# thomasahle/tinyknn

Measured on AMD Instinct MI355X. Metric: queries/sec at Recall10@10 on GloVe-100 angular (synthetic stand-in), IVF+4-bit PQ, build_probes=1, higher is better.
Workload: dtype int8 (saturating PQ sums) + f32 (tables, rescoring)

## Files before the change

include/tinyknn_hip.h:

```cpp
#ifndef TINYKNN_HIP_H
#define TINYKNN_HIP_H

#include <stdint.h>

#ifdef __cplusplus
extern "C" {
#endif

#define TK_ORDER_SSE 0
#define TK_ORDER_AVX 1

#define TK_OK 0
#define TK_ERR_ARG (-1)
#define TK_ERR_HIP (-2)
#define TK_ERR_STATE (-3)

const char *tk_last_error(void);
int tk_version(void);
int tk_device_count(void);
int tk_set_device(int device);


int tk_estimate_pq(const uint64_t *data, int64_t chunks, int M, const uint64_t *tables,
                   uint64_t *out, int signd, int order);
// ... 58 lines not shown
                             int q_pq_is_f64, int64_t nq, int k, int n_probes, int pass_1,
                             int64_t *out_ids_dev, void *stream);

int tk_index_set_pipeline(tk_index *ix, int depth);
int tk_index_join(tk_index *ix, void *stream);
int tk_index_set_coalesce(tk_index *ix, int n);
int tk_index_quiesce(tk_index *ix);

int tk_index_set_heap_mode(tk_index *ix, int mode);

int tk_index_set_scan_mode(tk_index *ix, int mode);

int tk_index_set_plain_scan(tk_index *ix, int mode);
int tk_index_plain_stats(tk_index *ix, int64_t *out8);
#define TK_OPT_SCAN_FORM 1
#define TK_OPT_RESCORE_FORM 2
#define TK_OPT_PLAIN_LIMIT 3
#define TK_OPT_REPLAY_LAZY 4
#define TK_OPT_REPLAY_COUNT 5
#define TK_OPT_REPLAY_TWIN 6
#define TK_OPT_TWIN_VOUCH 7
#define TK_OPT_PAIR_NQ 8
#define TK_OPT_LABELS24 9
int tk_index_set_option(tk_index *ix, int option, int value);
int tk_index_twin_table(tk_index *ix, int64_t *rows, int *w, int32_t *list_out, int32_t *off_out);

int tk_index_set_profiling(tk_index *ix, int on);
int tk_index_last_profile(tk_index *ix, float *ms8, double *scan_bytes, int *batches);

int tk_index_replay_stats(tk_index *ix, int64_t *out4);
int tk_measure_read_bandwidth(int64_t bytes, int reps, double *gbps);
int tk_measure_gather_bandwidth(int64_t table_bytes, int row_bytes, int64_t n_gather, int reps, double *gbps);
int tk_scan_exclusive_host(const void *in_host, void *out_host, int64_t n, int is64);

float *tk_index_alloc_data(tk_index *ix, int64_t N, int d);
int tk_index_synth_data(tk_index *ix, int64_t row0, int64_t n, uint64_t seed, const float *centres,
                        int n_centres, float sigma);
int tk_synth_rows(float *out, int64_t row0, int64_t n, int d, uint64_t seed, const float *centres,
                  int n_centres, float sigma);
int tk_index_build_dev(tk_index *ix, int normalise, const float *all_centers,
                       const float *search_centers, const float *ynorm2, int64_t C, int n_probes,
                       const double *R, int d_pad, int64_t *n_active_out);
int tk_index_export_lists(tk_index *ix, int64_t *list_sizes, uint64_t *codes, int64_t *ids);
int tk_index_export_centers(tk_index *ix, float *active_centers, uint64_t *center_codes);
int tk_index_read_rows(tk_index *ix, const int64_t *rows, int64_t n, float *out);

// ... 89 lines not shown
```

tinyknn_amd/_lib.py:

```python
import ctypes as C
import os

_HERE = os.path.dirname(os.path.abspath(__file__))

ORDER_SSE, ORDER_AVX = 0, 1


class TinyKnnHipError(RuntimeError):
    pass


def lib_path():
    return os.environ.get("TINYKNN_HIP_LIB", os.path.join(_HERE, "libtinyknn_hip.so"))


_lib = None
_lib_pid = None

_i64p = C.POINTER(C.c_int64)
_i32p = C.POINTER(C.c_int32)
_u64p = C.POINTER(C.c_uint64)
_u8p = C.POINTER(C.c_uint8)
_f32p = C.POINTER(C.c_float)
_f64p = C.POINTER(C.c_double)

OPT_SCAN_FORM, OPT_RESCORE_FORM, OPT_PLAIN_LIMIT, OPT_REPLAY_LAZY, OPT_REPLAY_COUNT, OPT_REPLAY_TWIN, OPT_TWIN_VOUCH = 1, 2, 3, 4, 5, 6, 7
OPT_PAIR_NQ, OPT_LABELS24 = 8, 9

SIGNATURES = {
    "tk_last_error": (C.c_char_p, []),
    "tk_version": (C.c_int, []),
    "tk_device_count": (C.c_int, []),
    "tk_set_device": (C.c_int, [C.c_int]),
    "tk_estimate_pq": (C.c_int, [_u64p, C.c_int64, C.c_int, _u64p, _u64p, C.c_int, C.c_int]),
    "tk_estimate_pq_batch": (C.c_int, [_u64p, C.c_int64, C.c_int, _u64p, C.c_int64, _u64p,
                                       C.c_int, C.c_int]),
    "tk_query_pq": (C.c_int, [_u64p, C.c_int64, C.c_int, C.c_int64, _u64p, _i64p, _i32p, C.c_int,
                              C.c_int, _i64p, C.c_int]),
    "tk_init_heap": (C.c_int, [_i64p, _i32p, C.c_int, C.c_int]),
    "tk_heap_insert": (C.c_int, [_i64p, _i32p, C.c_int, C.c_int64, C.c_int32]),
    "tk_heap_insert_is": (C.c_int, [_i64p, _i32p, C.c_int, C.c_int64, C.c_int32]),
    "tk_build_tables": (C.c_int, [_f32p, C.c_int, C.c_int, C.c_int, C.c_void_p, C.c_int, C.c_int64,
                                  C.c_double, C.c_double, C.c_int, _u8p, C.c_void_p, _f64p]),
    "tk_knn_brute1": (C.c_int64, [C.c_void_p, C.c_int, C.c_void_p, C.c_int, C.c_int64, C.c_int,
                                  C.c_int64, _i64p]),
    "tk_encode_pq": (C.c_int, [_f32p, C.c_int, C.c_int, C.c_void_p, C.c_int, C.c_int64, _u8p]),
    "tk_assign_lists": (C.c_int, [_f32p, C.c_int64, C.c_int, C.c_int, C.c_void_p, C.c_int,
                                  C.c_void_p, C.c_int64, C.c_int, _i64p]),
    "tk_codes_upload": (C.c_void_p, [_u64p, C.c_int64, C.c_int]),
    "tk_codes_free": (None, [C.c_void_p]),
# ... 151 lines not shown
```

tinyknn_amd/csrc/api_build.hip:

```cpp
#include "api_internal.h"

static int upload_rotation(tk_index *ix, const double *R, int d_pad)
{
    std::vector<double> rt((size_t)d_pad * ix->dq);
    for (int j = 0; j < ix->dq; j++)
        for (int t = 0; t < d_pad; t++) rt[(size_t)t * ix->dq + j] = R[(size_t)j * d_pad + t];
    TRY(ix->rot_t.ensure(rt.size() * 8));
    HIPCHECK(hipMemcpy(ix->rot_t.p, rt.data(), rt.size() * 8, hipMemcpyHostToDevice));
    ix->rot_d_pad = d_pad;
    return TK_OK;
}

extern "C" float *tk_index_alloc_data(tk_index *ix, int64_t N, int d)
{
    IXLOCK(ix);
    if (!ix || !ix->have_pq || N < 1 || d < 1) {
        fail(TK_ERR_ARG, "bad argument: tk_index_alloc_data (set_pq first, N >= 1, d >= 1)");
        return nullptr;
    }
    if (ix->data.ensure((size_t)N * d * 4) != TK_OK) return nullptr;
    ix->N = N;
    ix->d = d;
    ix->data_is_f64 = 0;
    ix->have_data = ix->have_centers = ix->have_lists = false;
    return ix->data.as<float>();
}

static int synth_centres(DevBuf &buf, const float *centres, int n_centres, int d, const float **dev)
{
    *dev = nullptr;
    if (!centres || n_centres <= 0) return TK_OK;
    TRY(buf.ensure((size_t)n_centres * d * 4));
    HIPCHECK(hipMemcpy(buf.p, centres, (size_t)n_centres * d * 4, hipMemcpyHostToDevice));
    *dev = buf.as<float>();
    return TK_OK;
}

extern "C" int tk_index_synth_data(tk_index *ix, int64_t row0, int64_t n, uint64_t seed,
                                   const float *centres, int n_centres, float sigma)
{
    IXLOCK(ix);
    ARGCHECK(ix && ix->data.p && ix->N > 0, "tk_index_alloc_data first");
    ARGCHECK(row0 >= 0 && n >= 0 && row0 + n <= ix->N, "row range");
    const float *cd = nullptr;
    TRY(synth_centres(ix->stage, centres, n_centres, ix->d, &cd));
    tk_launch_synth_rows(ix->data.as<float>() + row0 * ix->d, row0, n, ix->d, seed, cd, n_centres, sigma, 0);
    HIPCHECK(hipGetLastError());
// ... 170 lines not shown
    HIPCHECK(hipMemcpy(ix->ids_off.p, ioff.data(), (size_t)(L + 1) * 8, hipMemcpyHostToDevice));
    HIPCHECK(hipMemcpy(ix->list_n.p, sizes.data(), (size_t)L * 8, hipMemcpyHostToDevice));
    const size_t tiled_bytes = (size_t)tk_tiled_uint4s(coff[(size_t)L], P) * 16;
    TRY(ix->codes.ensure(tiled_bytes));
    HIPCHECK(hipMemset(ix->codes.p, 0, tiled_bytes));
    tk_launch_pack_lists(labels.as<uint8_t>(), M, rows2.as<int>(), ix->ids_off.as<int64_t>(),
                         ix->list_chunk_off.as<int64_t>(), ix->list_n.as<int64_t>(), (int)L, zero_code,
                         ix->codes.as<uint4>(), coff[(size_t)L], 0);
    tk_launch_widen_ids(rows2.as<int>(), T, ix->ids.as<int64_t>(), 0);
    HIPCHECK(hipGetLastError());
    ix->ids_unique = kp == 1;
    ix->labels24 = ix->N < 0x00ffffff;
    ix->have_ids32 = false;
    if (kp > 1) {
        TRY(ix->ids32.ensure((size_t)T * 4));
        HIPCHECK(hipMemcpyAsync(ix->ids32.p, rows2.p, (size_t)T * 4, hipMemcpyDeviceToDevice, 0));
        ix->have_ids32 = true;
    }
    HIPCHECK(hipDeviceSynchronize());
    ix->sharded = false; ix->rank = 0; ix->world = 1;
    ix->total_chunks = coff[(size_t)L];
    ix->total_ids = T;
    ix->max_list_chunks = (int)maxc;
    ix->have_centers = ix->have_lists = ix->have_data = true;
    TRY(build_twins(ix, N));
    if (n_active_out) *n_active_out = L;
    return TK_OK;
}

extern "C" int tk_index_shard_resident(tk_index *ix, const int32_t *owner, int rank, int world)
{
    IXLOCK(ix);
    ARGCHECK(ix && ix->have_lists && !ix->sharded, "a complete unsharded index");
    ARGCHECK(owner && world >= 1 && rank >= 0 && rank < world, "owner / rank / world");
    TRY(flush_pending(ix));
    HIPCHECK(hipDeviceSynchronize());
    const int64_t L = ix->n_lists;
    std::vector<int64_t> sizes((size_t)L), coff((size_t)L + 1, 0), loff((size_t)L + 1, 0);
    HIPCHECK(hipMemcpy(sizes.data(), ix->list_n.p, (size_t)L * 8, hipMemcpyDeviceToHost));
    for (int64_t i = 0; i < L; i++) {
        ARGCHECK(owner[i] >= 0 && owner[i] < world, "owner out of range");
        const int64_t c = (sizes[(size_t)i] + 15) / 16;
        coff[(size_t)i + 1] = coff[(size_t)i] + c;
        loff[(size_t)i + 1] = loff[(size_t)i] + (owner[i] == rank ? c : 0);
    }
    const int P = ix->M / 2;
// ... 36 lines not shown
    ix->n_lists = src->n_lists; ix->center_chunks = src->center_chunks; ix->d = src->d;
    ix->list_chunk_off.borrow(src->list_chunk_off);
    ix->list_n.borrow(src->list_n);
    ix->ids_off.borrow(src->ids_off);
    ix->ids.borrow(src->ids);
    ix->ids32.borrow(src->ids32);
    ix->have_ids32 = src->have_ids32;
    ix->labels24 = src->labels24;
    ix->twin_list.borrow(src->twin_list);
    ix->twin_off.borrow(src->twin_off);
    ix->twin_w = src->twin_w;
    ix->twin_unverified = src->twin_unverified;
    ix->twin_vouched = src->twin_vouched;
    ix->opt_replay_twin = src->opt_replay_twin;
    ix->total_chunks = src->total_chunks; ix->total_ids = src->total_ids;
    ix->max_list_chunks = src->max_list_chunks;
    ix->ids_unique = src->ids_unique;
    ix->cslots_i.borrow(src->cslots_i);
    ix->cslots_l.borrow(src->cslots_l);
    ix->c_chunk_off.borrow(src->c_chunk_off);
    ix->rot_t.borrow(src->rot_t);
    ix->rot_d_pad = src->rot_d_pad;
    ix->data.borrow(src->data);
    ix->N = src->N; ix->data_is_f64 = src->data_is_f64;
    ix->have_pq = ix->have_centers = ix->have_lists = ix->have_data = true;
    ix->plain_mode = src->plain_mode;
    const int64_t L = ix->n_lists;
    std::vector<int64_t> sizes((size_t)L), loff((size_t)L + 1, 0);
    bool ok = hipMemcpy(sizes.data(), src->list_n.p, (size_t)L * 8, hipMemcpyDeviceToHost) == hipSuccess;
    for (int64_t i = 0; ok && i < L; i++) {
        ok = owner[i] >= 0 && owner[i] < world;
        loff[(size_t)i + 1] = loff[(size_t)i] + (owner[i] == rank ? (sizes[(size_t)i] + 15) / 16 : 0);
    }
    const int P = ix->M / 2;
    const size_t bytes = (size_t)tk_tiled_uint4s(loff[(size_t)L], P) * 16;
    ok = ok && ix->owner.ensure((size_t)L * 4) == TK_OK && ix->local_chunk_off.ensure((size_t)(L + 1) * 8) == TK_OK &&
         ix->codes.ensure(bytes > 0 ? bytes : 16) == TK_OK;
    ok = ok && hipMemcpy(ix->owner.p, owner, (size_t)L * 4, hipMemcpyHostToDevice) == hipSuccess &&
         hipMemcpy(ix->local_chunk_off.p, loff.data(), (size_t)(L + 1) * 8, hipMemcpyHostToDevice) == hipSuccess &&
         hipMemset(ix->codes.p, 0, bytes > 0 ? bytes : 16) == hipSuccess;
    if (ok) {
        tk_launch_compact_tiled(src->codes.as<uint4>(), ix->codes.as<uint4>(), P, ix->list_chunk_off.as<int64_t>(),
                                ix->local_chunk_off.as<int64_t>(), (int)L, loff[(size_t)L], 0);
        ok = hipGetLastError() == hipSuccess && hipDeviceSynchronize() == hipSuccess;
    }
    if (!ok) {
// ... 305 lines not shown
```

tinyknn_amd/csrc/api_index.hip:

```cpp
#include "api_internal.h"


struct Pending;
static int batch_epilogue(const struct Pending &b, hipStream_t st);


extern "C" tk_index *tk_index_create(void)
{
    if (require_gpu() != TK_OK) return nullptr;
    tk_index *ix = new tk_index();
    ix->works.resize(1);
    const char *e = getenv("TINYKNN_PLAIN_SCAN");
    if (e && e[0] == '2') ix->plain_mode = 2;
    e = getenv("TINYKNN_PAIR_NQ");
    if (e && e[0] >= '0' && e[0] <= '9') ix->opt_pair_nq = atoi(e);
    return ix;
}

extern "C" void tk_index_destroy(tk_index *ix)
{
    if (!ix) return;
    (void)flush_pending(ix);
    (void)hipDeviceSynchronize();
    DevBuf *bufs[] = {&ix->pq_centers, &ix->active_centers, &ix->center_codes, &ix->list_chunk_off,
                      &ix->list_n, &ix->ids_off, &ix->ids, &ix->codes, &ix->ids32, &ix->data, &ix->cslots_i,
                      &ix->cslots_l, &ix->c_chunk_off, &ix->q, &ix->qpq, &ix->stage, &ix->owner,
                      &ix->local_chunk_off, &ix->rot_t, &ix->br_ynorm, &ix->br_vals, &ix->br_tau,
                      &ix->br_cand, &ix->br_count, &ix->br_out, &ix->br_q, &ix->br_sample, &ix->replay_counters,
                      &ix->twin_list, &ix->twin_off};
    for (DevBuf *b : bufs) b->release();
    for (Work &w : ix->works) w.release();
    if (ix->ev_in) (void)hipEventDestroy(ix->ev_in);
    for (auto &e : ix->evs) (void)hipEventDestroy(e);
    delete ix;
}

extern "C" int tk_index_set_pq(tk_index *ix, const float *centers, int dq, int dpb, int f_order,
                               double sqrt_n_blocks, int order)
{
    IXLOCK(ix);
    ARGCHECK(ix, "null index");
    ARGCHECK(dpb >= 1 && dpb <= 32 && dq % dpb == 0, "dq/dpb");
    ARGCHECK((dq / dpb) % 2 == 0, "number of blocks must be even");
    ARGCHECK(dq / dpb <= 512, "at most 512 blocks");
    ARGCHECK(order == TK_ORDER_SSE || order == TK_ORDER_AVX, "order");
    TRY(ix->pq_centers.ensure((size_t)16 * dq * 4));
    HIPCHECK(hipMemcpy(ix->pq_centers.p, centers, (size_t)16 * dq * 4, hipMemcpyHostToDevice));
    ix->dq = dq; ix->dpb = dpb; ix->M = dq / dpb; ix->f_order = f_order;
    ix->sqrt_nb = sqrt_n_blocks; ix->order = order;
    ix->have_pq = true;
    return TK_OK;
}
// ... 62 lines not shown
    TRY(t.where.ensure((size_t)label_bound * b * 4));
    TRY(ix->twin_list.ensure((size_t)T * w * 4));
    TRY(ix->twin_off.ensure((size_t)T * w * 4));
    HIPCHECK(hipMemsetAsync(t.cnt.p, 0, (size_t)label_bound * 4, 0));
    tk_launch_twin_fill(ix->ids32.as<int32_t>(), T, t.cnt.as<int>(), t.where.as<int>(), b,
                        ix->ids_off.as<int64_t>(), (int)ix->n_lists, ix->twin_list.as<int32_t>(),
                        ix->twin_off.as<int32_t>(), 0);
    HIPCHECK(hipGetLastError());
    HIPCHECK(hipDeviceSynchronize());
    if (!ix->sharded) {
        HIPCHECK(hipMemsetAsync(t.cnt.p, 0, 4, 0));
        tk_launch_twin_verify(ix->codes.as<uint4>(), ix->M / 2, ix->list_chunk_off.as<int64_t>(),
                              ix->ids_off.as<int64_t>(), (int)ix->n_lists, ix->twin_list.as<int32_t>(),
                              ix->twin_off.as<int32_t>(), w, T, t.cnt.as<int>(), 0);
        int bad = 0;
        HIPCHECK(hipMemcpy(&bad, t.cnt.p, 4, hipMemcpyDeviceToHost));
        if (bad) return TK_OK;
    }
    ix->twin_w = w;
    ix->twin_unverified = ix->sharded;
    return TK_OK;
}

int build_twins(tk_index *ix, int64_t label_bound)
{
    ix->twin_w = 0;
    ix->twin_unverified = false;
    ix->twin_list.release();
    ix->twin_off.release();
    const int64_t T = ix->total_ids;
    if (!ix->have_ids32 || ix->ids_unique || T <= 0 || T >= (1ll << 31) || label_bound <= 0 ||
        label_bound > 8 * T + 1024 || ix->n_lists >= (1ll << 31))
        return TK_OK;
    TwinScratch t;
    const int rc = build_twins_try(ix, label_bound, t);
    if (rc != TK_OK || ix->twin_w == 0) {
        ix->twin_w = 0;
        ix->twin_unverified = false;
        ix->twin_list.release();
        ix->twin_off.release();
    }
    if (rc != TK_OK) (void)hipGetLastError();
    return TK_OK;
}

extern "C" int tk_index_twin_table(tk_index *ix, int64_t *rows, int *w, int32_t *list_out, int32_t *off_out)
// ... 105 lines not shown

extern "C" int tk_index_set_lists_shard(tk_index *ix, const int64_t *list_sizes,
                                        const int32_t *owner, int rank, int world,
                                        const uint64_t *codes_owned, const int64_t *ids)
{
    IXLOCK(ix);
    ARGCHECK(owner, "owner");
    ARGCHECK(world >= 1 && rank >= 0 && rank < world, "rank/world");
    return set_lists_impl(ix, list_sizes, codes_owned, ids, owner, rank, world);
}

extern "C" int tk_index_set_data(tk_index *ix, const void *data, int data_is_f64, int64_t N,
                                 int d)
{
    IXLOCK(ix);
    ARGCHECK(ix && ix->have_centers, "set_centers first");
    ARGCHECK(d == ix->d, "data dimension differs from the centres'");
    ARGCHECK(N >= 1, "N");
    const size_t esz = data_is_f64 ? 8 : 4;
    TRY(ix->data.ensure((size_t)N * d * esz));
    HIPCHECK(hipMemcpy(ix->data.p, data, (size_t)N * d * esz, hipMemcpyHostToDevice));
    ix->N = N;
    ix->data_is_f64 = data_is_f64;
    ix->have_data = true;
    return TK_OK;
}


int make_plan(const tk_index *ix, int k, int n_probes, int pass_1, Plan &p)
{
    ARGCHECK(ix && ix->have_pq && ix->have_centers && ix->have_lists && ix->have_data,
             "index not fully populated (pq, centers, lists, data)");
    ARGCHECK(k >= 1 && n_probes >= 1, "k and n_probes must be >= 1");
    int64_t kc = n_probes < ix->n_lists ? n_probes : ix->n_lists;
    int64_t rescore = 2 * kc + 10 < ix->n_lists ? 2 * kc + 10 : ix->n_lists;
    int64_t R = pass_1 > 0 ? pass_1 : (int64_t)(n_probes + 1) * k + 1;
    ARGCHECK(R * 12 + 16 <= 64 * 1024 && rescore * 12 + 16 <= 64 * 1024,
             "heap larger than 64 KiB of LDS (pass_1 <= 5460)");
    ARGCHECK(R * (ix->data_is_f64 ? 16 : 12) + (int64_t)ix->d * (ix->data_is_f64 ? 8 : 4) + 16 <= 64 * 1024,
             "rescoring tile larger than 64 KiB of LDS");
    p.kc = (int)kc; p.rescore = (int)rescore; p.R = (int)R; p.S = (int)kc;
    p.cap = (int64_t)kc * ix->max_list_chunks;
    if (p.cap < 1) p.cap = 1;
    ARGCHECK(p.cap < (1ll << 31), "probed chunk range overflows int32");
    p.cap_min = (p.cap + 15) / 16 * 16;
    p.ccap_min = (ix->center_chunks + 15) / 16 * 16;
// ... 619 lines not shown
                                        slot_loff, p.S, ix->ids.as<int64_t>(),
                                        w.heap_idx.as<int64_t>(), w.heap_val.as<int32_t>(), p.R, 1,
                                        0, plain ? repeat_flag : nullptr, w.mins.as<uint8_t>(), p.cap_min,
                                        ix->ids32.as<int32_t>(), st, slot_exact, qlim))
            return fail(TK_ERR_HIP, "hipFuncSetAttribute(LDS size) failed");
        if (plain) {
            rescan_flagged(ix, w, q0, nq, p, st);
            tk_launch_heap_replay_packed(w.dist.as<uint4>(), p.cap, nq, slot_prefix, slot_n, slot_loff,
                                         p.S, ix->ids.as<int64_t>(), w.heap_idx.as<int64_t>(),
                                         w.heap_val.as<int32_t>(), p.R, 1, 0, repeat_flag, 1, 1, st);
        }
    } else if (packed_ok) {
        tk_launch_heap_replay_packed(w.dist.as<uint4>(), p.cap, nq, slot_prefix, slot_n, slot_loff,
                                     p.S, ix->ids.as<int64_t>(), w.heap_idx.as<int64_t>(),
                                     w.heap_val.as<int32_t>(), p.R, 1, 0, nullptr, 0, 1, st);
    } else {
        tk_launch_heap_fill(w.heap_idx.as<int64_t>(), w.heap_val.as<int32_t>(), nq * p.R, 127, st);
        tk_launch_heap_replay(w.dist.as<uint4>(), p.cap, nq, slot_prefix, slot_n, slot_loff, p.S,
                              ix->ids.as<int64_t>(), w.heap_idx.as<int64_t>(),
                              w.heap_val.as<int32_t>(), p.R, 1, 0, nullptr, st);
    }
    TRY(pf.mark(st));
    tk_launch_rescore(q_dev, 0, ix->d, ix->data.p, ix->data_is_f64, ix->N, w.heap_idx.as<int64_t>(), p.R, nq, k, 1,
                      out_dev, nullptr, st, ix->opt_rescore_form, q2, out2);
    TRY(pf.mark(st));
    return TK_OK;
}

struct Pending {
    Work *w;
    const float *q_dev;
    int64_t nq;
    int k;
    Plan p;
    int64_t *out_dev;
    bool units;
    bool plain;
    bool coarse_launched;
    int64_t *host_out;
    bool host_out_kernel;
    hipEvent_t user_ev;
    Prof pf;
    hipStream_t st, sf, sl;
    struct Sub {
        int64_t *out_dev;
        int64_t nq;
        int64_t *host_out;
// ... 574 lines not shown
{
    IXLOCK(ix);
    ARGCHECK(ix, "null index");
    ARGCHECK(mode >= 0 && mode <= 3, "mode");
    TRY(flush_pending(ix));
    ix->heap_mode = mode;
    return TK_OK;
}

extern "C" int tk_index_set_option(tk_index *ix, int option, int value)
{
    IXLOCK(ix);
    ARGCHECK(ix, "null index");
    TRY(flush_pending(ix));
    switch (option) {
    case TK_OPT_SCAN_FORM:
        ARGCHECK(value >= 0 && value <= 2, "TK_OPT_SCAN_FORM: 0, 1 or 2");
        ix->opt_scan_form = value;
        return TK_OK;
    case TK_OPT_RESCORE_FORM:
        ARGCHECK(value >= 0 && value <= 2, "TK_OPT_RESCORE_FORM: 0, 1 or 2");
        ix->opt_rescore_form = value;
        return TK_OK;
    case TK_OPT_PLAIN_LIMIT:
        ix->opt_plain_limit = value;
        return TK_OK;
    case TK_OPT_PAIR_NQ:
        ARGCHECK(value >= 0, "TK_OPT_PAIR_NQ: >= 0");
        ix->opt_pair_nq = value;
        return TK_OK;
    case TK_OPT_LABELS24:
        ix->opt_labels24 = value != 0;
        return TK_OK;
    case TK_OPT_REPLAY_COUNT:
        ix->opt_replay_count = value != 0;
        if (value) {
            TRY(ix->replay_counters.ensure(64));
            HIPCHECK(hipMemset(ix->replay_counters.p, 0, 64));
        }
        return TK_OK;
    case TK_OPT_REPLAY_LAZY:
        ARGCHECK(value >= -1 && value <= 1, "TK_OPT_REPLAY_LAZY: -1, 0 or 1");
        ix->opt_replay_lazy = value;
        return TK_OK;
    case TK_OPT_REPLAY_TWIN:
        ARGCHECK(value == 0 || value == 1, "TK_OPT_REPLAY_TWIN: 0 or 1");
// ... 137 lines not shown
```

tinyknn_amd/csrc/api_internal.h:

```cpp
#pragma once
#include <algorithm>
#include <cmath>
#include <mutex>
#include <stdlib.h>
#include <string.h>
#include <stdio.h>
#include <string>
#include <vector>

#include "../../include/tinyknn_hip.h"
#include "kernels.h"

int tk_fail(int code, const std::string &msg);
static inline int fail(int code, const std::string &msg) { return tk_fail(code, msg); }

#define HIPCHECK(x)                                                                          \
    do {                                                                                     \
        hipError_t e_ = (x);                                                                 \
        if (e_ != hipSuccess) {                                                              \
            char b_[512];                                                                    \
            snprintf(b_, sizeof b_, "%s failed: %s (%s:%d)", #x, hipGetErrorString(e_),      \
                     __FILE__, __LINE__);                                                    \
            return fail(TK_ERR_HIP, b_);                                                     \
        }                                                                                    \
// ... 131 lines not shown
    DevBuf list_chunk_off, list_n, ids_off, ids, codes, ids32;
    bool have_ids32 = false;
    bool labels24 = false;
    int opt_labels24 = 1;
    DevBuf twin_list, twin_off;
    int twin_w = 0;
    bool twin_unverified = false, twin_vouched = false;
    int opt_replay_twin = 1;
    int64_t total_chunks = 0, total_ids = 0;
    int max_list_chunks = 0;
    bool ids_unique = false;
    int heap_mode = 0;
    int opt_pair_nq = 8192;
    bool have_pq = false, have_centers = false, have_lists = false, have_data = false;
    DevBuf owner, local_chunk_off;
    DevBuf rot_t;
    DevBuf br_ynorm, br_vals, br_tau, br_cand, br_count, br_out, br_q, br_sample;
    int rot_d_pad = 0;
    int rank = 0, world = 1;
    bool sharded = false;
    DevBuf data;
    int64_t N = 0;
    int data_is_f64 = 0;
    DevBuf cslots_i, cslots_l, c_chunk_off, q, qpq, stage;
    int scan_mode = 0;
    int opt_scan_form = 0;
    int opt_rescore_form = 2;
    int opt_plain_limit = 0x7fffffff;
    DevBuf replay_counters;
    bool opt_replay_count = false;
    int opt_replay_lazy = -1;
    bool flat_plain_ok = true;
    int plain_state = 0;
    int plain_skip = 0;
    int plain_backoff = 256;
    int plain_wait = 0;
    bool capturing = false;
    int plain_mode = 0;
    bool host_out_kernel = false;
    std::vector<Work> works;
    int depth = 1;
    uint64_t calls = 0;
    std::vector<hipStream_t> lat_streams;
    hipEvent_t ev_in = nullptr;
    std::vector<struct Pending *> pending;
    uint64_t ev_seq = 0;
// ... 32 lines not shown
    size_t base = 0;
    int evi = 0;
    int set = -1;
    bool plain_marked = false;
    int mark(hipStream_t st)
    {
        if (evs) HIPCHECK(hipEventRecord((*evs)[base + (size_t)evi++], st));
        return TK_OK;
    }
    int mark_plain(int which, hipStream_t st)
    {
        if (evs) {
            HIPCHECK(hipEventRecord((*evs)[base + 8 + (size_t)which], st));
            plain_marked = true;
        }
        return TK_OK;
    }
};

inline const uint4 *tables_of(const Work &w) { return w.tables.as<uint4>(); }

int flush_pending(tk_index *ix);
int build_twins(tk_index *ix, int64_t label_bound);
bool twin_replay(const tk_index *ix, const struct Plan &p);
int make_plan(const tk_index *ix, int k, int n_probes, int pass_1, Plan &p);
bool plain_env_on();
int plain_k(const tk_index *ix, int64_t nq, const Plan &p);
size_t plain_desc_bytes(const tk_index *ix, int64_t nq, const Plan &p);
double workspace_bytes();
bool coarse_units(const tk_index *ix, int64_t nq);
int stage_tables(tk_index *ix, Work &w, const void *qpq_dev, int qpq_f64, int64_t nq, hipStream_t st, Prof &pf,
                 bool plain = false, TkSecond qpq2 = TkSecond(), int64_t row0 = 0);
TkScanJob coarse_job(const tk_index *ix, const Work &w, const Plan &p);
int plain_blocks();
int shard_plain_blocks();
void launch_coarse_scan(tk_index *ix, Work &w, int64_t nq, const Plan &p, hipStream_t st,
                        const uint4 *tables = nullptr);
int coarse_replay_probes(tk_index *ix, Work &w, const float *q_dev, int64_t nq, const Plan &p,
                         int64_t *probes_out, hipStream_t st, Prof &pf, TkSecond q2 = TkSecond(),
                         const TkSlotsOut *slots = nullptr, int *slots_written = nullptr);
void coarse_slots(tk_index *ix, Work &w, const int64_t *probes, int64_t nq, const Plan &p,
                  int *pair_count, const int *owner, int me, hipStream_t st, bool plain = false);
int stage_coarse_rest(tk_index *ix, Work &w, const float *q_dev, int64_t nq, const Plan &p,
                      int *pair_count, const int *owner, int me, hipStream_t st, Prof &pf,
                      bool plain = false, TkSecond q2 = TkSecond());
int stage_back(tk_index *ix, Work &w, const float *q_dev, int64_t q0, int64_t nq, int k,
// ... 4 lines not shown
```

tinyknn_amd/csrc/kernels.h:

```cpp
#pragma once
#include <hip/hip_runtime.h>
#include <stdint.h>

#define TK_ORDER_SSE 0
#define TK_ORDER_AVX 1

static inline size_t tk_unit_prefix_ints(int64_t n_lists)
{
    return (size_t)(((n_lists + 1 + 31) / 32 + 1) * 32 + 8 * 32);
}

static inline int64_t tk_tiled_uint4s(int64_t chunks, int P)
{
    return ((chunks + 7) / 8) * 8 * (int64_t)P;
}

void tk_launch_retile(const uint4 *src_ref, uint4 *dst_tiled, int64_t chunks, int P,
                      hipStream_t s);

void tk_launch_scan_flat(const uint4 *codes, int64_t chunks, int M, const uint4 *tables,
                         int64_t nq, uint4 *out, int64_t out_stride, uint8_t *mins,
                         int64_t min_stride, int signd, int order, hipStream_t s);

void tk_launch_scan_probes(const uint4 *codes, int M, const uint4 *tables, int64_t nq,
// ... 127 lines not shown
void tk_launch_build_tables(const float *centers, int dq, int dpb, int f_order, const void *q,
                            int q_is_f64, int64_t nq, double aux0, double aux1, int signd,
                            uint8_t *tables, void *shift, double *scale, hipStream_t s, TkSecond q2 = TkSecond(),
                            const TkTablesExtra *extra = nullptr);

struct TkSlotsOut {
    int64_t n_lists;
    const int64_t *list_chunk_off, *list_n, *ids_off;
    int *slot_prefix;
    int64_t *slot_chunk0;
    int *slot_n;
    int64_t *slot_label_off;
    unsigned char *repeat_flag;
    int *pair_count;
    const int *owner;
    int me;
    const int *qlim;
    int R;
    int *slot_exact, *pair_count2, *plain0, *pair_count3;
};
int tk_launch_rescore(const void *q, int q_is_f64, int d, const void *rows, int rows_is_f64,
                      int64_t n_rows, const int64_t *cand, int R, int64_t nq, int k, int strip,
                      int64_t *out, int *out_count, hipStream_t s, int form = 2, TkSecond q2 = TkSecond(),
                      TkSecond out2 = TkSecond(), const TkSlotsOut *slots = nullptr);

void tk_launch_make_slots(const int64_t *probes, const int *probe_count, int kc, int64_t nq,
                          int64_t n_lists, const int64_t *list_chunk_off, const int64_t *list_n,
                          const int64_t *ids_off, int *slot_prefix, int64_t *slot_chunk0,
                          int *slot_n, int64_t *slot_label_off, unsigned char *repeat_flag,
                          int *pair_count, const int *owner, int me, hipStream_t s,
                          const int *qlim = nullptr, int R = 0, int *slot_exact = nullptr,
                          int *pair_count2 = nullptr, int *plain0 = nullptr, int *pair_count3 = nullptr);

void tk_launch_pairs_scan(int *count, const int64_t *list_chunk_off, int64_t n_lists, int *pair_off,
                          int *unit_prefix, int *cursor, int *pair_q, hipStream_t s);

int tk_scan_exclusive64(void *tmp, size_t *tmp_bytes, const long long *in, long long *out, int64_t n,
                        hipStream_t s);
int tk_launch_shard_positions(const int64_t *probes, const int *slot_prefix, int S, int64_t nq,
                              int64_t n_lists, const int *owner, int me, int W, int64_t qh,
                              int64_t C, int *spos, int *rpos, int *flag, long long *usage,
                              long long *lens, long long *P, void *tmp, size_t tmp_bytes,
                              hipStream_t s);
void tk_launch_shard_pairs_fill(const int64_t *probes, int S, int64_t nq, int64_t n_lists,
                                const int *owner, int me, const int *spos, const int *pair_off,
                                int *cursor, int *pair_q, int *pair_f0, hipStream_t s, int s_lo = 0,
                                int s_hi = 0x7fffffff, const uint8_t *sel = nullptr, int want = 0,
// ... 64 lines not shown
```

tinyknn_amd/csrc/rescore.hip:

```cpp
#include <stdlib.h>
#include <string.h>

#include "kernels.h"

#ifndef TK_NT
#define TK_NT 0
#endif

template <typename T, typename TY>
__device__ __forceinline__ T sqdist_row(const TY *__restrict__ y, const T *xs, int d)
{
    constexpr int L = 16 / (int)sizeof(T);
    T acc[L];
#pragma unroll
    for (int l = 0; l < L; l++) acc[l] = 0;
    int i = 0;
    for (; d - i >= 4 * L; i += 4 * L) {
        T df[4 * L];
#pragma unroll
        for (int t = 0; t < 4 * L; t++) df[t] = (T)(TK_NT ? __builtin_nontemporal_load(y + i + t) : y[i + t]) - xs[i + t];
#pragma unroll
        for (int l = 0; l < L; l++) {
            T ab3 = df[3 * L + l] * df[3 * L + l] + acc[l];
            T ab2 = df[2 * L + l] * df[2 * L + l] + ab3;
// ... 141 lines not shown
    if (!plain_ok) e = S;
    bool head = false;
    if (so.slot_exact) {
        const int E = (so.R + 15) >> 4;
        const int first_len = __shfl(acc, 0, 64);
        head = plain_ok && e_walk == 1 && first_len > E;
        const int at_e = e > 0 ? __shfl(acc, e - 1, 64) : 0;
        if (lane == 0) {
            so.slot_exact[qi] = head ? 0 : e;
            so.plain0[qi] = head ? E : at_e;
        }
    }
    if (so.pair_count && act && !(so.owner && so.owner[cl] != so.me)) {
        if (head && lane == 0) {
            atomicAdd(&so.pair_count3[cl], 1);
            atomicAdd(&so.pair_count2[cl], 1);
        } else {
            atomicAdd(lane < e ? &so.pair_count[cl] : &so.pair_count2[cl], 1);
        }
    }
    if (lane == 0 && so.repeat_flag) so.repeat_flag[qi] = wrapped;
}

template <int TILE>
__global__ __launch_bounds__(64) void rescore_staged_kernel(const float *__restrict__ q, int d,
                                                            const float *__restrict__ rows,
                                                            int64_t n_rows,
                                                            const int64_t *__restrict__ cand, int R,
                                                            int k, int strip, int64_t *__restrict__ out,
                                                            int *__restrict__ out_count, int stride4,
                                                            const float *__restrict__ q_b, int64_t q_na,
                                                            int64_t *__restrict__ out_b, int64_t out_na,
                                                            const TkSlotsOut *__restrict__ so_dev)
{
    const bool have_slots = so_dev != nullptr;
    extern __shared__ __attribute__((aligned(16))) unsigned char smem[];
    int64_t *cs = (int64_t *)smem;
    float *ds = (float *)(smem + (((size_t)R * 8 + 15) & ~(size_t)15));
    float *xs = ds + ((R + 3) & ~3);
    float4 *tile = (float4 *)(xs + ((d + 3) & ~3));
    const int tid = threadIdx.x;
    const int64_t qi = blockIdx.x;
    const int64_t *c = cand + qi * R;
    const float *qrow = (q_b && qi >= q_na) ? q_b + (qi - q_na) * d : q + qi * d;
    for (int t = tid; t < d; t += 64) xs[t] = qrow[t];
    int nc = 0;
    for (int t0 = 0; t0 < R; t0 += 64) {
        const int t = t0 + tid;
        const int64_t id = t < R ? c[t] : -1;
        const bool keep = t < R && (!strip || id != -1);
        const uint64_t m = __builtin_amdgcn_ballot_w64(keep);
        const int before = __builtin_popcountll(m & ((1ull << tid) - 1ull));
        if (keep) cs[nc + before] = id;
        nc += __builtin_popcountll(m);
    }
    __syncthreads();
    int64_t *o = (out_b && qi >= out_na) ? out_b + (qi - out_na) * k : out + qi * k;
    if (nc <= k) {
        for (int t = tid; t < k; t += 64) o[t] = t < nc ? cs[t] : -1;
        if (tid == 0 && out_count) out_count[qi] = nc;
        if (have_slots) slots_epilogue(*so_dev, qi, k, tid, tid < nc ? cs[tid < k ? tid : 0] : -1);
        return;
    }
    const int d4 = d >> 2;
    const int lpr_log = d4 <= 16 ? 4 : (d4 <= 32 ? 5 : 6);
    const int rr = tid >> lpr_log, pc = tid & ((1 << lpr_log) - 1), rpi = 64 >> lpr_log;
    for (int t0 = 0; t0 < nc; t0 += TILE) {
        const int nt = nc - t0 < TILE ? nc - t0 : TILE;
        if (pc < d4)
            for (int r0 = rr; r0 < nt; r0 += 16 * rpi) {
                float4 v[16];
#pragma unroll
                for (int u = 0; u < 16; u++) {
                    const int r = r0 + u * rpi;
                    int64_t id = cs[t0 + (r < nt ? r : nt - 1)];
                    if (id < 0) id += n_rows;
                    v[u] = ((const float4 *)(rows + id * (int64_t)d))[pc];
                }
#pragma unroll
                for (int u = 0; u < 16; u++) {
                    const int r = r0 + u * rpi;
                    tile[(r < nt ? r : TILE) * stride4 + pc] = v[u];
                }
            }
        __syncthreads();
        if (tid < nt) ds[t0 + tid] = sqdist_row_lds(tile + tid * stride4, xs, d);
        __syncthreads();
    }
    int64_t *ps = (int64_t *)(tile + (TILE + 1) * stride4);
    for (int t = tid; t < nc; t += 64) {
        const float dv = ds[t];
        int rank = 0;
        for (int u = 0; u < nc; u++) {
            const float du = ds[u];
            rank += (du < dv) || (du == dv && u < t);
        }
        if (rank < k) {
            o[rank] = cs[t];
            if (have_slots) ps[rank] = cs[t];
        }
    }
    if (tid == 0 && out_count) out_count[qi] = k;
    if (have_slots) {
        __syncthreads();
        slots_epilogue(*so_dev, qi, k, tid, tid < k ? ps[tid] : -1);
    }
}

int tk_launch_rescore(const void *q, int q_is_f64, int d, const void *rows, int rows_is_f64,
                      int64_t n_rows, const int64_t *cand, int R, int64_t nq, int k, int strip,
                      int64_t *out, int *out_count, hipStream_t s, int form, TkSecond q2, TkSecond out2,
                      const TkSlotsOut *slots)
{
    if (nq == 0 || k == 0) return 0;
    const bool dbl = q_is_f64 || rows_is_f64;
    size_t lds = (size_t)R * 8 + ((size_t)R + d) * (dbl ? 8 : 4) + 16;
    dim3 grid((unsigned)nq), block(R <= 64 ? 64 : 128);
    const int staged = form < 0 || form > 2 ? 2 : form;
    if (!dbl && staged && d % 4 == 0 && d <= 256 && R <= 256 ) {
        const int stride4 = (d / 4) | 1;
        const int tile_rows = staged == 2 ? 32 : 64;
        const bool fuse = slots != nullptr && k <= 64;
        const TkSlotsOut *so = fuse ? slots : nullptr;
        const size_t slds = (((size_t)R * 8 + 15) & ~(size_t)15) +
                            (size_t)(((R + 3) & ~3) + ((d + 3) & ~3)) * 4 + (size_t)(tile_rows + 1) * stride4 * 16 +
                            (fuse ? (size_t)k * 8 : 0);
        if (slds <= 64 * 1024) {
            if (tile_rows == 32)
                hipLaunchKernelGGL(rescore_staged_kernel<32>, grid, dim3(64), slds, s, (const float *)q, d,
                                   (const float *)rows, n_rows, cand, R, k, strip, out, out_count, stride4,
                                   (const float *)q2.b, q2.n_a, (int64_t *)out2.b, out2.n_a, so);
            else
                hipLaunchKernelGGL(rescore_staged_kernel<64>, grid, dim3(64), slds, s, (const float *)q, d,
                                   (const float *)rows, n_rows, cand, R, k, strip, out, out_count, stride4,
                                   (const float *)q2.b, q2.n_a, (int64_t *)out2.b, out2.n_a, so);
            return fuse ? 1 : 0;
        }
    }
    if (!dbl)
        hipLaunchKernelGGL((rescore_kernel<float, float, float>), grid, block, lds, s,
                           (const float *)q, d, (const float *)rows, n_rows, cand, R, k, strip, out,
                           out_count, (const float *)q2.b, q2.n_a, (int64_t *)out2.b, out2.n_a);
    else if (rows_is_f64 && q_is_f64)
        hipLaunchKernelGGL((rescore_kernel<double, double, double>), grid, block, lds, s,
                           (const double *)q, d, (const double *)rows, n_rows, cand, R, k, strip,
                           out, out_count, (const double *)q2.b, q2.n_a, (int64_t *)out2.b, out2.n_a);
    else if (rows_is_f64)
        hipLaunchKernelGGL((rescore_kernel<double, double, float>), grid, block, lds, s,
                           (const float *)q, d, (const double *)rows, n_rows, cand, R, k, strip, out,
                           out_count, (const float *)q2.b, q2.n_a, (int64_t *)out2.b, out2.n_a);
    else
// ... 97 lines not shown
```

Measured before the change: 25.40 million.

## Prefilter rescore candidates with int8 compact rows and error bounds

Builds an int8-quantized copy of every data row, storing a per-row scale and a rigorous bound on the quantization error. During rescoring, candidates are first scored against these compact rows to get lower and upper distance bounds. The k-th smallest upper bound becomes a threshold, and any candidate whose lower bound exceeds it is dropped before the full f32 row gather. This cuts f32 gather traffic in rescoring, at the cost of extra device memory, an O(R^2) rank pass and an extra compact-row read per candidate.

```diff
diff --git a/include/tinyknn_hip.h b/include/tinyknn_hip.h
--- a/include/tinyknn_hip.h
+++ b/include/tinyknn_hip.h
@@ -104,6 +104,7 @@
 #define TK_OPT_TWIN_VOUCH 7
 #define TK_OPT_PAIR_NQ 8
 #define TK_OPT_LABELS24 9
+#define TK_OPT_RESCORE_PREFILTER 10
 int tk_index_set_option(tk_index *ix, int option, int value);
 int tk_index_twin_table(tk_index *ix, int64_t *rows, int *w, int32_t *list_out, int32_t *off_out);
 
diff --git a/tinyknn_amd/_lib.py b/tinyknn_amd/_lib.py
--- a/tinyknn_amd/_lib.py
+++ b/tinyknn_amd/_lib.py
@@ -25,7 +25,7 @@
 _f64p = C.POINTER(C.c_double)
 
 OPT_SCAN_FORM, OPT_RESCORE_FORM, OPT_PLAIN_LIMIT, OPT_REPLAY_LAZY, OPT_REPLAY_COUNT, OPT_REPLAY_TWIN, OPT_TWIN_VOUCH = 1, 2, 3, 4, 5, 6, 7
-OPT_PAIR_NQ, OPT_LABELS24 = 8, 9
+OPT_PAIR_NQ, OPT_LABELS24, OPT_RESCORE_PREFILTER = 8, 9, 10
 
 SIGNATURES = {
     "tk_last_error": (C.c_char_p, []),
diff --git a/tinyknn_amd/csrc/api_build.hip b/tinyknn_amd/csrc/api_build.hip
--- a/tinyknn_amd/csrc/api_build.hip
+++ b/tinyknn_amd/csrc/api_build.hip
@@ -23,6 +23,8 @@
     ix->d = d;
     ix->data_is_f64 = 0;
     ix->have_data = ix->have_centers = ix->have_lists = false;
+    ix->have_compact = false;
+    ix->compact.release();
     return ix->data.as<float>();
 }
 
@@ -239,6 +241,7 @@
     ix->total_chunks = coff[(size_t)L];
     ix->total_ids = T;
     ix->max_list_chunks = (int)maxc;
+    TRY(build_compact(ix));
     ix->have_centers = ix->have_lists = ix->have_data = true;
     TRY(build_twins(ix, N));
     if (n_active_out) *n_active_out = L;
@@ -321,6 +324,8 @@
     ix->rot_t.borrow(src->rot_t);
     ix->rot_d_pad = src->rot_d_pad;
     ix->data.borrow(src->data);
+    ix->compact.borrow(src->compact);
+    ix->have_compact = src->have_compact;
     ix->N = src->N; ix->data_is_f64 = src->data_is_f64;
     ix->have_pq = ix->have_centers = ix->have_lists = ix->have_data = true;
     ix->plain_mode = src->plain_mode;
diff --git a/tinyknn_amd/csrc/api_index.hip b/tinyknn_amd/csrc/api_index.hip
--- a/tinyknn_amd/csrc/api_index.hip
+++ b/tinyknn_amd/csrc/api_index.hip
@@ -27,7 +27,7 @@
                       &ix->cslots_l, &ix->c_chunk_off, &ix->q, &ix->qpq, &ix->stage, &ix->owner,
                       &ix->local_chunk_off, &ix->rot_t, &ix->br_ynorm, &ix->br_vals, &ix->br_tau,
                       &ix->br_cand, &ix->br_count, &ix->br_out, &ix->br_q, &ix->br_sample, &ix->replay_counters,
-                      &ix->twin_list, &ix->twin_off};
+                      &ix->twin_list, &ix->twin_off, &ix->compact};
     for (DevBuf *b : bufs) b->release();
     for (Work &w : ix->works) w.release();
     if (ix->ev_in) (void)hipEventDestroy(ix->ev_in);
@@ -136,6 +136,29 @@
     return TK_OK;
 }
 
+int build_compact(tk_index *ix)
+{
+    ix->have_compact = false;
+    ix->compact.release();
+    const int stride = tk_compact_stride(ix->d);
+    if (ix->data_is_f64 || stride == 0 || ix->N <= 0 || !ix->data.p) return TK_OK;
+    void *p = nullptr;
+    const size_t bytes = (size_t)ix->N * stride;
+    const hipError_t e = hipMalloc(&p, bytes);
+    if (e == hipErrorOutOfMemory) {
+        (void)hipGetLastError();
+        return TK_OK;
+    }
+    HIPCHECK(e);
+    ix->compact.p = p;
+    ix->compact.cap = bytes;
+    tk_launch_compact_rows(ix->data.as<float>(), ix->N, ix->d, ix->compact.as<unsigned char>(), 0);
+    HIPCHECK(hipGetLastError());
+    HIPCHECK(hipDeviceSynchronize());
+    ix->have_compact = true;
+    return TK_OK;
+}
+
 int build_twins(tk_index *ix, int64_t label_bound)
 {
     ix->twin_w = 0;
@@ -287,6 +310,7 @@
     HIPCHECK(hipMemcpy(ix->data.p, data, (size_t)N * d * esz, hipMemcpyHostToDevice));
     ix->N = N;
     ix->data_is_f64 = data_is_f64;
+    TRY(build_compact(ix));
     ix->have_data = true;
     return TK_OK;
 }
@@ -952,7 +976,8 @@
     }
     TRY(pf.mark(st));
     tk_launch_rescore(q_dev, 0, ix->d, ix->data.p, ix->data_is_f64, ix->N, w.heap_idx.as<int64_t>(), p.R, nq, k, 1,
-                      out_dev, nullptr, st, ix->opt_rescore_form, q2, out2);
+                      out_dev, nullptr, st, ix->opt_rescore_form, q2, out2, nullptr,
+                      ix->have_compact && ix->opt_rescore_prefilter ? ix->compact.p : nullptr);
     TRY(pf.mark(st));
     return TK_OK;
 }
@@ -1573,6 +1598,10 @@
         ARGCHECK(value >= 0 && value <= 2, "TK_OPT_RESCORE_FORM: 0, 1 or 2");
         ix->opt_rescore_form = value;
         return TK_OK;
+    case TK_OPT_RESCORE_PREFILTER:
+        ARGCHECK(value == 0 || value == 1, "TK_OPT_RESCORE_PREFILTER: 0 or 1");
+        ix->opt_rescore_prefilter = value;
+        return TK_OK;
     case TK_OPT_PLAIN_LIMIT:
         ix->opt_plain_limit = value;
         return TK_OK;
diff --git a/tinyknn_amd/csrc/api_internal.h b/tinyknn_amd/csrc/api_internal.h
--- a/tinyknn_amd/csrc/api_internal.h
+++ b/tinyknn_amd/csrc/api_internal.h
@@ -177,6 +177,9 @@
     DevBuf data;
     int64_t N = 0;
     int data_is_f64 = 0;
+    DevBuf compact;
+    bool have_compact = false;
+    int opt_rescore_prefilter = 1;
     DevBuf cslots_i, cslots_l, c_chunk_off, q, qpq, stage;
     int scan_mode = 0;
     int opt_scan_form = 0;
@@ -255,6 +258,7 @@
 
 int flush_pending(tk_index *ix);
 int build_twins(tk_index *ix, int64_t label_bound);
+int build_compact(tk_index *ix);
 bool twin_replay(const tk_index *ix, const struct Plan &p);
 int make_plan(const tk_index *ix, int k, int n_probes, int pass_1, Plan &p);
 bool plain_env_on();
diff --git a/tinyknn_amd/csrc/kernels.h b/tinyknn_amd/csrc/kernels.h
--- a/tinyknn_amd/csrc/kernels.h
+++ b/tinyknn_amd/csrc/kernels.h
@@ -173,7 +173,9 @@
 int tk_launch_rescore(const void *q, int q_is_f64, int d, const void *rows, int rows_is_f64,
                       int64_t n_rows, const int64_t *cand, int R, int64_t nq, int k, int strip,
                       int64_t *out, int *out_count, hipStream_t s, int form = 2, TkSecond q2 = TkSecond(),
-                      TkSecond out2 = TkSecond(), const TkSlotsOut *slots = nullptr);
+                      TkSecond out2 = TkSecond(), const TkSlotsOut *slots = nullptr, const void *compact = nullptr);
+int tk_compact_stride(int d);
+void tk_launch_compact_rows(const float *X, int64_t N, int d, unsigned char *out, hipStream_t s);
 
 void tk_launch_make_slots(const int64_t *probes, const int *probe_count, int kc, int64_t nq,
                           int64_t n_lists, const int64_t *list_chunk_off, const int64_t *list_n,
diff --git a/tinyknn_amd/csrc/rescore.hip b/tinyknn_amd/csrc/rescore.hip
--- a/tinyknn_amd/csrc/rescore.hip
+++ b/tinyknn_amd/csrc/rescore.hip
@@ -187,16 +187,155 @@
     if (lane == 0 && so.repeat_flag) so.repeat_flag[qi] = wrapped;
 }
 
-template <int TILE>
-__global__ __launch_bounds__(64) void rescore_staged_kernel(const float *__restrict__ q, int d,
-                                                            const float *__restrict__ rows,
-                                                            int64_t n_rows,
-                                                            const int64_t *__restrict__ cand, int R,
-                                                            int k, int strip, int64_t *__restrict__ out,
-                                                            int *__restrict__ out_count, int stride4,
-                                                            const float *__restrict__ q_b, int64_t q_na,
-                                                            int64_t *__restrict__ out_b, int64_t out_na,
-                                                            const TkSlotsOut *__restrict__ so_dev)
+__global__ __launch_bounds__(256) void compact_rows_kernel(const float *__restrict__ X, int64_t N, int d, int stride,
+                                                           unsigned char *__restrict__ out)
+{
+    const int64_t r = (int64_t)blockIdx.x * blockDim.x + threadIdx.x;
+    if (r >= N) return;
+    const float4 *x4 = (const float4 *)(X + r * d);
+    float m = 0.f;
+    bool fin = true;
+    for (int i = 0; i < (d >> 2); i++) {
+        const float4 v = x4[i];
+        fin = fin && isfinite(v.x) && isfinite(v.y) && isfinite(v.z) && isfinite(v.w);
+        m = fmaxf(m, fmaxf(fmaxf(fabsf(v.x), fabsf(v.y)), fmaxf(fabsf(v.z), fabsf(v.w))));
+    }
+    const float sc = fin ? m / 127.f : 0.f;
+    double err = 0.0;
+    uint4 *o = (uint4 *)(out + r * stride);
+    const int np = stride >> 4;
+    uint4 last = make_uint4(0, 0, 0, 0);
+    for (int p = 0; p < np; p++) {
+        unsigned w[4] = {0u, 0u, 0u, 0u};
+        for (int j = 0; j < 16; j++) {
+            const int i = p * 16 + j;
+            if (i >= d) break;
+            const float x = X[r * d + i];
+            float c = sc > 0.f ? rintf(x / sc) : 0.f;
+            c = fminf(fmaxf(c, -127.f), 127.f);
+            const float y = sc * c;
+            const double df = (double)x - (double)y;
+            err += df * df;
+            w[j >> 2] |= ((unsigned)(int)c & 0xffu) << (8 * (j & 3));
+        }
+        const uint4 v = make_uint4(w[0], w[1], w[2], w[3]);
+        if (p < np - 1) o[p] = v;
+        else last = v;
+    }
+    const double ed = sqrt(err) * (1.0 + 0x1p-40);
+    float e = (float)ed;
+    if ((double)e < ed) e = __uint_as_float(__float_as_uint(e) + 1u);
+    if (!fin) e = INFINITY;
+    last.z = __float_as_uint(sc);
+    last.w = __float_as_uint(e);
+    o[np - 1] = last;
+}
+
+int tk_compact_stride(int d)
+{
+    return d % 4 == 0 && d <= 256 ? (d + 8 + 127) / 128 * 128 : 0;
+}
+
+void tk_launch_compact_rows(const float *X, int64_t N, int d, unsigned char *out, hipStream_t s)
+{
+    if (N <= 0) return;
+    hipLaunchKernelGGL(compact_rows_kernel, dim3((unsigned)((N + 255) / 256)), dim3(256), 0, s, X, N, d,
+                       tk_compact_stride(d), out);
+}
+
+__device__ __forceinline__ int prefilter(const unsigned char *__restrict__ compact, int cstride, int64_t n_rows,
+                                         int64_t *cs, int nc, int k, float *hi, float *lo, const float *xs, int d,
+                                         int tid)
+{
+    const float eps = 0x1p-12f, da_abs = 0x1p-50f, tiny = 0x1p-100f;
+    const int np = cstride >> 4;
+    const int lpr_log = np <= 8 ? 3 : (np <= 16 ? 4 : 5);
+    const int P = 1 << lpr_log, rpp = 64 >> lpr_log;
+    const int rr = tid >> lpr_log, pc = tid & (P - 1);
+    bool bad = false;
+    const int src = (tid & ~(P - 1)) + np - 1;
+    constexpr int U = 8;
+    for (int t0 = 0; t0 < nc; t0 += U * rpp) {
+        uint4 v[U];
+#pragma unroll
+        for (int u = 0; u < U; u++) {
+            const int t = t0 + u * rpp + rr;
+            int64_t id = cs[t < nc ? t : nc - 1];
+            if (id < 0) id += n_rows;
+            v[u] = ((const uint4 *)(compact + id * (int64_t)cstride))[pc < np ? pc : np - 1];
+        }
+#pragma unroll
+        for (int u = 0; u < U; u++) {
+            const int t = t0 + u * rpp + rr;
+            const bool act = t < nc && pc < np;
+            const float sc = __uint_as_float((unsigned)__shfl((int)v[u].z, src, 64));
+            const float e = __uint_as_float((unsigned)__shfl((int)v[u].w, src, 64));
+            float acc = 0.f;
+            const unsigned w[4] = {v[u].x, v[u].y, v[u].z, v[u].w};
+#pragma unroll
+            for (int g = 0; g < 4; g++) {
+                const int i = pc * 16 + g * 4;
+                if (act && i < d) {
+                    const float4 x = *(const float4 *)(xs + i);
+                    const float xv[4] = {x.x, x.y, x.z, x.w};
+#pragma unroll
+                    for (int b = 0; b < 4; b++) {
+                        const float y = sc * (float)(int)(signed char)(w[g] >> (8 * b));
+                        const float df = y - xv[b];
+                        acc = df * df + acc;
+                    }
+                }
+            }
+#pragma unroll
+            for (int o = 1; o < 64; o <<= 1)
+                if (o < P) acc += __shfl_xor(acc, o, 64);
+            if (act && pc == 0) {
+                const float da = sqrtf(acc);
+                bad = bad || !isfinite(da) || !isfinite(e);
+                const float ah = (da * (1.f + eps) + da_abs) + e;
+                const float al = (da * (1.f - eps) - da_abs) - e;
+                hi[t] = ah * ah * (1.f + eps) + tiny;
+                lo[t] = al > 0.f ? al * al * (1.f - eps) : 0.f;
+            }
+        }
+    }
+    __syncthreads();
+    if (__builtin_amdgcn_ballot_w64(bad)) return nc;
+    float T = 0.f;
+    for (int t = tid; t < nc; t += 64) {
+        const float hv = hi[t];
+        int rank = 0;
+        for (int u = 0; u < nc; u++) {
+            const float hu = hi[u];
+            rank += (hu < hv) || (hu == hv && u < t);
+        }
+        if (rank == k - 1) T = hv;
+    }
+#pragma unroll
+    for (int o = 1; o < 64; o <<= 1) T = fmaxf(T, __shfl_xor(T, o, 64));
+    int ns = 0;
+    for (int t0 = 0; t0 < nc; t0 += 64) {
+        const int t = t0 + tid;
+        const bool keep = t < nc && lo[t] <= T;
+        const int64_t id = t < nc ? cs[t] : 0;
+        const uint64_t m = __builtin_amdgcn_ballot_w64(keep);
+        const int before = __builtin_popcountll(m & ((1ull << tid) - 1ull));
+        if (keep) cs[ns + before] = id;
+        ns += __builtin_popcountll(m);
+    }
+    __syncthreads();
+    return ns;
+}
+
+template <int TILE, bool PRE>
+__device__ __forceinline__ void rescore_staged_body(const float *__restrict__ q, int d,
+                                                    const float *__restrict__ rows, int64_t n_rows,
+                                                    const int64_t *__restrict__ cand, int R, int k, int strip,
+                                                    int64_t *__restrict__ out, int *__restrict__ out_count,
+                                                    int stride4, const float *__restrict__ q_b, int64_t q_na,
+                                                    int64_t *__restrict__ out_b, int64_t out_na,
+                                                    const TkSlotsOut *__restrict__ so_dev,
+                                                    const unsigned char *__restrict__ compact, int cstride)
 {
     const bool have_slots = so_dev != nullptr;
     extern __shared__ __attribute__((aligned(16))) unsigned char smem[];
@@ -227,6 +366,7 @@
         if (have_slots) slots_epilogue(*so_dev, qi, k, tid, tid < nc ? cs[tid < k ? tid : 0] : -1);
         return;
     }
+    if (PRE) nc = prefilter(compact, cstride, n_rows, cs, nc, k, ds, (float *)tile, xs, d, tid);
     const int d4 = d >> 2;
     const int lpr_log = d4 <= 16 ? 4 : (d4 <= 32 ? 5 : 6);
     const int rr = tid >> lpr_log, pc = tid & ((1 << lpr_log) - 1), rpi = 64 >> lpr_log;
@@ -272,10 +412,38 @@
     }
 }
 
+template <int TILE>
+__global__ __launch_bounds__(64) void rescore_staged_kernel(const float *__restrict__ q, int d,
+                                                            const float *__restrict__ rows,
+                                                            int64_t n_rows,
+                                                            const int64_t *__restrict__ cand, int R,
+                                                            int k, int strip, int64_t *__restrict__ out,
+                                                            int *__restrict__ out_count, int stride4,
+                                                            const float *__restrict__ q_b, int64_t q_na,
+                                                            int64_t *__restrict__ out_b, int64_t out_na,
+                                                            const TkSlotsOut *__restrict__ so_dev)
+{
+    rescore_staged_body<TILE, false>(q, d, rows, n_rows, cand, R, k, strip, out, out_count, stride4, q_b, q_na,
+                                     out_b, out_na, so_dev, nullptr, 0);
+}
+
+__global__ __launch_bounds__(64) void rescore_pruned_kernel(const float *__restrict__ q, int d,
+                                                            const float *__restrict__ rows, int64_t n_rows,
+                                                            const int64_t *__restrict__ cand, int R, int k,
+                                                            int strip, int64_t *__restrict__ out,
+                                                            int *__restrict__ out_count, int stride4,
+                                                            const float *__restrict__ q_b, int64_t q_na,
+                                                            int64_t *__restrict__ out_b, int64_t out_na,
+                                                            const unsigned char *__restrict__ compact, int cstride)
+{
+    rescore_staged_body<32, true>(q, d, rows, n_rows, cand, R, k, strip, out, out_count, stride4, q_b, q_na,
+                                  out_b, out_na, nullptr, compact, cstride);
+}
+
 int tk_launch_rescore(const void *q, int q_is_f64, int d, const void *rows, int rows_is_f64,
                       int64_t n_rows, const int64_t *cand, int R, int64_t nq, int k, int strip,
                       int64_t *out, int *out_count, hipStream_t s, int form, TkSecond q2, TkSecond out2,
-                      const TkSlotsOut *slots)
+                      const TkSlotsOut *slots, const void *compact)
 {
     if (nq == 0 || k == 0) return 0;
     const bool dbl = q_is_f64 || rows_is_f64;
@@ -287,11 +455,20 @@
         const int tile_rows = staged == 2 ? 32 : 64;
         const bool fuse = slots != nullptr && k <= 64;
         const TkSlotsOut *so = fuse ? slots : nullptr;
+        const bool pre = compact != nullptr && tile_rows == 32 && !fuse;
+        size_t tile_b = (size_t)(tile_rows + 1) * stride4 * 16;
+        if (pre && tile_b < (size_t)R * 4) tile_b = ((size_t)R * 4 + 15) & ~(size_t)15;
         const size_t slds = (((size_t)R * 8 + 15) & ~(size_t)15) +
-                            (size_t)(((R + 3) & ~3) + ((d + 3) & ~3)) * 4 + (size_t)(tile_rows + 1) * stride4 * 16 +
+                            (size_t)(((R + 3) & ~3) + ((d + 3) & ~3)) * 4 + tile_b +
                             (fuse ? (size_t)k * 8 : 0);
+        const unsigned char *cp = (const unsigned char *)compact;
+        const int cstride = tk_compact_stride(d);
         if (slds <= 64 * 1024) {
-            if (tile_rows == 32)
+            if (pre)
+                hipLaunchKernelGGL(rescore_pruned_kernel, grid, dim3(64), slds, s, (const float *)q, d,
+                                   (const float *)rows, n_rows, cand, R, k, strip, out, out_count, stride4,
+                                   (const float *)q2.b, q2.n_a, (int64_t *)out2.b, out2.n_a, cp, cstride);
+            else if (tile_rows == 32)
                 hipLaunchKernelGGL(rescore_staged_kernel<32>, grid, dim3(64), slds, s, (const float *)q, d,
                                    (const float *)rows, n_rows, cand, R, k, strip, out, out_count, stride4,
                                    (const float *)q2.b, q2.n_a, (int64_t *)out2.b, out2.n_a, so);
```

Result: slower. 23.07 million, median of 6 (-9.1%).
